# bytedance/particle-sfm

Measured on AMD Instinct MI355X. Metric: trajectory-points/s, higher is better.
Workload: dtype f32 sampling + f64 positions; 1 GPU; configs[1]: synthetic 100x(1920x1080) flow pairs, sample_ratio=2, flow_check + chaining + occlusion + id assignment, 1 sequence per GPU; frames=101, height=1080, width=1920, trajectories=2073277, parallelism=sequence-per-gpu x1, world_size=1

## Files before the change

### particle-sfm_amd/csrc/psfm_finalize.hip

```cpp
#include <cstring>
#include <stdio.h>
#include <rocprim/device/device_radix_sort.hpp>
#include <rocprim/device/device_scan.hpp>

#include "psfm_device.h"
#include "psfm_internal.h"

#define PSFM_BLOCK 256

__device__ __forceinline__ void psfm_collect_alive_body(
    const int* __restrict__ birth_frame, const int* __restrict__ birth_idx, PsfmCounters* __restrict__ ctr,
    PsfmShard* __restrict__ shards, unsigned long long* __restrict__ fin_keys, int* __restrict__ fin_lanes, int cap,
    int shard_cap, int last_time, int shift_b, int shift_d)
{
    __shared__ int s_cnt[PSFM_BLOCK / PSFM_WAVE];
    __shared__ int s_base;
    const int n_lanes = min(ctr->n_lanes, cap);
    if ((int)(blockIdx.x * PSFM_BLOCK) >= n_lanes) return;
    const int i = blockIdx.x * PSFM_BLOCK + threadIdx.x;
    int bf = -1;
    if (i < n_lanes) bf = birth_frame[i];
    const bool pending = bf <= -2;
    const bool alive = (bf >= 0) | pending;
    const int my_last = pending ? last_time - 1 : last_time;
// ... 276 lines not shown
        r[u] = t < lj ? log[(int64_t)(bj + t) * cap + col] : make_double2(0.0, 0.0);
    }
    if (tid < TILE_J) s_off[tid] = id0 + tid < n ? psfm_track_offset(pl, off, id0 + tid, hb, hl) : 0;
    for (int k0 = 0; k0 < maxlen; k0 += TILE_K) {
#pragma unroll
        for (int u = 0; u < NLD; ++u) tile[j][q + u * (PSFM_BLOCK / TILE_J)] = r[u];
        __syncthreads();
        if (k0 + TILE_K < maxlen) {
#pragma unroll
            for (int u = 0; u < NLD; ++u) {
                const int t = k0 + TILE_K + q + u * (PSFM_BLOCK / TILE_J);
                r[u] = t < lj ? log[(int64_t)(bj + t) * cap + col] : make_double2(0.0, 0.0);
            }
        }
        const int kk = tid & (TILE_K - 1);
        for (int jj = tid / TILE_K; jj < TILE_J; jj += PSFM_BLOCK / TILE_K) {
            const int t = k0 + kk;
            if (t < s_len[jj]) out[s_off[jj] + t] = tile[jj][kk];
        }
        __syncthreads();
    }
}

__global__ __launch_bounds__(PSFM_BLOCK) void psfm_gather_kernel(const double2* __restrict__ log, int64_t cap,
                                                                 const int* __restrict__ lanes,
                                                                 const int* __restrict__ birth,
                                                                 const int* __restrict__ len,
                                                                 const int64_t* __restrict__ off, int64_t n,
                                                                 double2* __restrict__ out, PsfmPlan pl)
{
    psfm_gather_body(log, cap, lanes, birth, len, off, n, out, pl);
}

__global__ __launch_bounds__(PSFM_BLOCK) void psfm_gather_delta_kernel(const float2* __restrict__ dlog, int64_t cap,
                                                                       const int* __restrict__ lanes,
                                                                       const int* __restrict__ birth,
                                                                       const int* __restrict__ len,
                                                                       const int64_t* __restrict__ off, int64_t n,
                                                                       const void* __restrict__ keys, int use32, int shift_b,
                                                                       int GW, int ratio, double2* __restrict__ out, PsfmPlan pl)
{
    __shared__ float2 dtile[TILE_J][TILE_K + 1];
    __shared__ double2 tile[TILE_J][TILE_K + 1];
    __shared__ double2 s_pos[TILE_J];
    __shared__ int s_lane[TILE_J], s_birth[TILE_J], s_len[TILE_J];
    __shared__ int64_t s_off[TILE_J];
    __shared__ int s_maxlen;
    const int tid = threadIdx.x;
    const int64_t id0 = (int64_t)blockIdx.x * TILE_J;
    int hb = 0, hl = 0;
    if (tid == 0) s_maxlen = 0;
    __syncthreads();
    if (tid < TILE_J) {
        const int64_t id = id0 + tid;
        const bool ok = id < n;
        int b = 0, l = 0, idx = -1;
        const int my_lane = ok ? lanes[id] : 0;
        if (ok) psfm_track_header(pl, birth, len, id, &b, &l, &idx);
        hb = b; hl = l;
        s_lane[tid] = my_lane;
        s_birth[tid] = b;
        s_len[tid] = l;
        if (ok) {
            atomicMax(&s_maxlen, l);
            if (idx < 0) {
                const unsigned long long mask = (1ull << shift_b) - 1ull;
                idx = (int)((use32 ? (unsigned long long)((const unsigned*)keys)[id] : ((const unsigned long long*)keys)[id]) & mask);
            }
            const int gy = idx / GW, gx = idx - gy * GW;
            s_pos[tid] = make_double2((double)(gx * ratio), (double)(gy * ratio));
        }
    }
    __syncthreads();
    const int maxlen = s_maxlen;
    const int j = tid & (TILE_J - 1);
    const int q = tid / TILE_J;
    constexpr int NLD = TILE_K * TILE_J / PSFM_BLOCK;
    const int lj = s_len[j];
    const int64_t col = s_lane[j];
    const int bj = s_birth[j];
    float2 r[NLD];
#pragma unroll
    for (int u = 0; u < NLD; ++u) {
        const int t = q + u * (PSFM_BLOCK / TILE_J);
        r[u] = (t >= 1 && t < lj) ? dlog[(int64_t)(bj + t - 1) * cap + col] : make_float2(0.f, 0.f);
    }
    if (tid < TILE_J) s_off[tid] = id0 + tid < n ? psfm_track_offset(pl, off, id0 + tid, hb, hl) : 0;
    for (int k0 = 0; k0 < maxlen; k0 += TILE_K) {
#pragma unroll
        for (int u = 0; u < NLD; ++u) dtile[j][q + u * (PSFM_BLOCK / TILE_J)] = r[u];
        __syncthreads();
        if (k0 + TILE_K < maxlen) {
#pragma unroll
            for (int u = 0; u < NLD; ++u) {
                const int t = k0 + TILE_K + q + u * (PSFM_BLOCK / TILE_J);
                r[u] = (t < lj) ? dlog[(int64_t)(bj + t - 1) * cap + col] : make_float2(0.f, 0.f);
            }
        }
        if (tid < TILE_J) {
            double2 pos = s_pos[tid];
            const int l = s_len[tid];
            float2 f[TILE_K];
#pragma unroll
            for (int k = 0; k < TILE_K; ++k) f[k] = dtile[tid][k];
#pragma unroll
            for (int k = 0; k < TILE_K; ++k) {
                const int t = k0 + k;
                if (t >= 1 && t < l) { pos.x = pos.x + (double)f[k].x; pos.y = pos.y + (double)f[k].y; }
                tile[tid][k] = pos;
            }
            s_pos[tid] = pos;
        }
        __syncthreads();
        const int kk = tid & (TILE_K - 1);
        for (int jj = tid / TILE_K; jj < TILE_J; jj += PSFM_BLOCK / TILE_K) {
            const int t = k0 + kk;
            if (t < s_len[jj]) out[s_off[jj] + t] = tile[jj][kk];
        }
        __syncthreads();
    }
}

static PsfmKeyFmt psfm_key_fmt(const PsfmTrackDims& d, unsigned* end_bit)
{
    PsfmKeyFmt f;
    f.shift_b = d.shift_b; f.shift_d = d.shift_d;
    const long long lmax = (long long)d.n_flows + 1;
    const long long tri_max = lmax * (lmax + 1) / 2 + lmax;
    int tri_bits = 1;
    while ((1ll << tri_bits) <= tri_max) ++tri_bits;
    f.use32 = (tri_bits + d.shift_b <= 32) ? 1 : 0;
    int tbits = 1;
    while ((1ll << tbits) < (long long)d.n_flows + 2) ++tbits;
    *end_bit = f.use32 ? (unsigned)(tri_bits + d.shift_b) : (unsigned)(d.shift_d + tbits);
    return f;
}

static bool psfm_own_sort(const PsfmKeyFmt& fmt, int64_t n)
{
    static const int on = getenv("PSFM_FIN_SORT") ? atoi(getenv("PSFM_FIN_SORT")) : 1;
    return on && fmt.use32 && n < (1ll << 31);
}
static bool psfm_records_in_first_half(const PsfmTrackDims& d, int64_t n)
{
    unsigned end_bit = 0;
    const PsfmKeyFmt fmt = psfm_key_fmt(d, &end_bit);
    return psfm_own_sort(fmt, n) && (psfm_sort_pairs32_passes(end_bit) % 2 == 0);
}

static psfm_status psfm_finalize_sorted(psfm_ctx* c, const PsfmTrackDims& d, int64_t n, int64_t npts, bool delta_log, hipStream_t s)
{
    psfm_status st;
// ... 31 lines not shown
    pl.birth_w = c->res_birth.as<int>(); pl.len_w = c->res_len.as<int>(); pl.off_w = c->res_off.as<int64_t>();
    if (plan_on && ng <= PSFM_PLAN_MAX_GROUPS && n < (1ll << 31)) {
        if ((st = c->scan_tmp.ensure((sizeof(int64_t) + sizeof(int)) * (size_t)ng)) != PSFM_OK) return st;
        int64_t* goff = c->scan_tmp.as<int64_t>();
        int* gstart = (int*)(goff + ng);
        const void* had = c->fin_marks.p;
        if ((st = c->fin_marks.ensure(sizeof(int) * (size_t)PSFM_PLAN_MAX_GROUPS)) != PSFM_OK) return st;
        if (!c->fin_marks_clean || had != c->fin_marks.p)
            PSFM_HIP(hipMemsetAsync(c->fin_marks.p, 0xff, sizeof(int) * (size_t)PSFM_PLAN_MAX_GROUPS, s));
        c->fin_marks_clean = false;
        hipLaunchKernelGGL(psfm_group_bounds_kernel, dim3((unsigned)((n + PSFM_BLOCK - 1) / PSFM_BLOCK)), dim3(PSFM_BLOCK), 0, s,
                           (const void*)c->sort_keys.p, n, fmt.use32, d.shift_b, d.shift_d, c->fin_marks.as<int>());
        hipLaunchKernelGGL(psfm_group_plan_kernel, dim3(1), dim3(PSFM_PLAN_BLOCK), 0, s, c->fin_marks.as<int>(), gstart, goff, (int)ng, n,
                           c->res_off.as<int64_t>() + n);
        PSFM_HIP(hipGetLastError());
        c->fin_marks_clean = true;
        pl.gstart = gstart; pl.goff = goff;
    } else {
        if ((st = c->scan_tmp.ensure(sizeof(int64_t) * (n + 1))) != PSFM_OK) return st;
        if (fmt.use32)
            hipLaunchKernelGGL(psfm_decode32_kernel, dim3((unsigned)((n + 1 + PSFM_BLOCK - 1) / PSFM_BLOCK)), dim3(PSFM_BLOCK), 0, s,
                               c->sort_keys.as<unsigned>(), n, d.shift_b, c->res_birth.as<int>(), c->res_len.as<int>(),
                               c->scan_tmp.as<int64_t>());
        else
            hipLaunchKernelGGL(psfm_decode_kernel, dim3((unsigned)((n + 1 + PSFM_BLOCK - 1) / PSFM_BLOCK)), dim3(PSFM_BLOCK), 0, s,
                               c->sort_keys.as<unsigned long long>(), n, d.shift_b, d.shift_d, c->res_birth.as<int>(),
                               c->res_len.as<int>(), c->scan_tmp.as<int64_t>());
        PSFM_HIP(hipGetLastError());
        PSFM_HIP(rocprim::exclusive_scan(c->sort_tmp.p, scan_bytes, c->scan_tmp.as<int64_t>(), c->res_off.as<int64_t>(),
                                         (int64_t)0, (size_t)(n + 1), rocprim::plus<int64_t>(), s));
    }
    c->res_n_points = npts;
    if ((st = c->res_xy.ensure(sizeof(double2) * (size_t)(npts > 0 ? npts : 1))) != PSFM_OK) return st;
    if (delta_log)
        hipLaunchKernelGGL(psfm_gather_delta_kernel, dim3((unsigned)((n + TILE_J - 1) / TILE_J)), dim3(PSFM_BLOCK), 0, s,
                           c->log.as<float2>(), d.cap, c->sort_lanes.as<int>(), c->res_birth.as<int>(),
                           c->res_len.as<int>(), c->res_off.as<int64_t>(), n, (const void*)c->sort_keys.p, fmt.use32,
                           d.shift_b, d.GW, d.ratio, c->res_xy.as<double2>(), pl);
    else
        hipLaunchKernelGGL(psfm_gather_kernel, dim3((unsigned)((n + TILE_J - 1) / TILE_J)), dim3(PSFM_BLOCK), 0, s,
                           c->log.as<double2>(), d.cap, c->sort_lanes.as<int>(), c->res_birth.as<int>(),
                           c->res_len.as<int>(), c->res_off.as<int64_t>(), n, c->res_xy.as<double2>(), pl);
    PSFM_HIP(hipGetLastError());
    return PSFM_OK;
}

psfm_status psfm_finalize(psfm_ctx* c, const PsfmTrackDims& d, hipStream_t s)
{
    PsfmCounters* ctr = c->counters.as<PsfmCounters>();
    PsfmShard* shards = c->shards.as<PsfmShard>();
    hipLaunchKernelGGL(psfm_collect_alive_kernel, dim3((unsigned)((d.cap + PSFM_BLOCK - 1) / PSFM_BLOCK)), dim3(PSFM_BLOCK),
                       0, s, c->birth_frame.as<int>(), c->birth_idx.as<int>(), ctr, shards,
                       c->fin_keys.as<unsigned long long>(), c->fin_lanes.as<int>(), (int)d.cap, d.shard_cap,
                       d.n_flows, d.shift_b, d.shift_d);
    PSFM_HIP(hipGetLastError());
    PsfmCounters* hc = (PsfmCounters*)c->host_pinned;
    PsfmShard* hs = (PsfmShard*)((char*)c->host_pinned + 512);
    PSFM_HIP(hipMemcpyAsync(hc, ctr, sizeof(PsfmCounters), hipMemcpyDeviceToHost, s));
    PSFM_HIP(hipMemcpyAsync(hs, shards, sizeof(PsfmShard) * PSFM_NSHARD, hipMemcpyDeviceToHost, s));
    PSFM_HIP(hipStreamSynchronize(s));
    PsfmShardOffsets so;
    int64_t n = 0, npts = 0;
    bool over = hc->overflow != 0;
    for (int k = 0; k < PSFM_NSHARD; ++k) npts += hs[k].points;
    for (int k = 0; k < PSFM_NSHARD; ++k) {
        if (hs[k].fin_cnt > d.shard_cap) over = true;
        so.count[k] = hs[k].fin_cnt > d.shard_cap ? d.shard_cap : hs[k].fin_cnt;
        so.start[k] = n;
        n += so.count[k];
    }
    if (over || hc->n_lanes > d.cap) {
// ... 334 lines not shown
```

### particle-sfm_amd/point_trajectory/_hip.py

```python
import ctypes
import os

_PKG = os.path.dirname(os.path.dirname(os.path.abspath(__file__)))
LIB_PATH = os.environ.get("PSFM_HIP_LIB", os.path.join(_PKG, "lib", "libpsfm_hip.so"))

PSFM_OK, PSFM_ERR_ARG, PSFM_ERR_HIP, PSFM_ERR_CAPACITY, PSFM_ERR_SOLVER = 0, 1, 2, 3, 4
PROF_KINDS = {"flow_check": 0, "chain_step": 1, "respawn": 2, "solver": 3, "finalize": 4}

EXPORTS = [
    "psfm_last_error", "psfm_version", "psfm_device_count", "psfm_ctx_create", "psfm_ctx_destroy",
    "psfm_ctx_set_capacity", "psfm_flow_check", "psfm_grid_sample", "psfm_optimize_location", "psfm_track",
    "psfm_connect",
    "psfm_result_device", "psfm_result_copy", "psfm_result_solve_stats", "psfm_ctx_set_profiling",
    "psfm_profile_get", "psfm_ctx_set_chain_mode", "psfm_window_sample", "psfm_result_filter", "psfm_result_filtered_copy",
    "psfm_ctx_set_solver", "psfm_solver_counters", "psfm_traj_to_matches", "psfm_matches_copy",
    "psfm_shard_begin", "psfm_shard_step", "psfm_shard_solve_export", "psfm_shard_solve_control", "psfm_shard_solve_restore",
    "psfm_shard_solve_writeback", "psfm_shard_solve_record", "psfm_shard_finish", "psfm_result_keys",
    "psfm_shard_solve_control_async", "psfm_shard_window_state", "psfm_shard_peek_stall", "psfm_shard_frame",
    "psfm_shard_solve_control_chain_async", "psfm_shard_solve_poll", "psfm_shard_solve_local", "psfm_shard_solve_redo_local", "psfm_connect_batch", "psfm_solver_launches", "psfm_ctx_set_resident_budget", "psfm_resident_capacity", "psfm_load_flo_stack",
    "psfm_path_consistency_eval", "psfm_sort_records",
    "psfm_shard_peer_area", "psfm_shard_peer_epoch", "psfm_shard_peer_open", "psfm_shard_peer_connect", "psfm_shard_solve_blocks", "psfm_shard_solve_peer",
    "psfm_labels_begin", "psfm_labels_merge_window", "psfm_labels_finish", "psfm_labels_device", "psfm_labels_copy", "psfm_labels_to_matches",
]

# ... 77 lines not shown
    L.psfm_labels_to_matches.argtypes = [vp, i32, i32, i32, ctypes.POINTER(i64), ctypes.POINTER(i64), ctypes.POINTER(i64), vp]
    L.psfm_shard_begin.argtypes = [vp, i32, i32, i32, i32, i64, i64, i32, vp, i64, vp]
    L.psfm_shard_step.argtypes = [vp, vp, vp, i32, vp]
    L.psfm_shard_solve_export.argtypes = [vp, vp, vp, vp, vp, i32, i32, i32, vp, vp]
    L.psfm_shard_frame.argtypes = [vp, vp, vp, vp, vp, vp, i32, i32, vp, vp]
    L.psfm_shard_solve_control.argtypes = [vp, i32, i32, i32, vp, ctypes.POINTER(ctypes.c_int32), ctypes.POINTER(ctypes.c_int32),
                                           ctypes.POINTER(SolveStats), vp]
    L.psfm_shard_solve_control_async.argtypes = [vp, i32, i32, vp, vp]
    L.psfm_shard_solve_control_chain_async.argtypes = [vp, i32, i32, vp, vp]
    L.psfm_shard_solve_poll.argtypes = [vp, ctypes.POINTER(ctypes.c_int32), ctypes.POINTER(SolveStats), vp]
    L.psfm_shard_solve_local.argtypes = [vp, vp, vp, vp, vp, i32, i32, vp]
    L.psfm_shard_peer_area.argtypes = [vp, ctypes.POINTER(vp), vp, vp]
    L.psfm_shard_peer_open.argtypes = [vp, vp, i32, ctypes.POINTER(vp)]
    L.psfm_shard_peer_epoch.argtypes = [vp, ctypes.POINTER(ctypes.c_uint32), i32, vp]
    L.psfm_shard_peer_connect.argtypes = [vp, i32, i32, ctypes.POINTER(vp), ctypes.POINTER(ctypes.c_int32)]
    L.psfm_shard_solve_blocks.argtypes = [vp, ctypes.POINTER(ctypes.c_int32)]
    L.psfm_shard_solve_peer.argtypes = [vp, vp, vp, vp, vp, i32, ctypes.c_uint32, vp]
    L.psfm_shard_solve_redo_local.argtypes = [vp, vp, vp, vp, vp, i32, i32, ctypes.POINTER(SolveStats), vp]
    L.psfm_shard_window_state.argtypes = [vp, i32, i32, ctypes.POINTER(SolveStats), ctypes.POINTER(ctypes.c_int32), vp]
    L.psfm_shard_peek_stall.argtypes = [vp, ctypes.POINTER(ctypes.c_int32)]
    L.psfm_shard_solve_restore.argtypes = [vp, i32, vp]
    L.psfm_shard_solve_writeback.argtypes = [vp, i32, ctypes.POINTER(SolveStats), vp]
    L.psfm_shard_solve_record.argtypes = [vp, ctypes.POINTER(SolveStats)]
    L.psfm_shard_finish.argtypes = [vp, ctypes.POINTER(TrackInfo), vp]
    L.psfm_result_keys.argtypes = [vp, i32, i32, vp, vp]
    L.psfm_profile_get.argtypes = [vp, i32, ctypes.POINTER(f64), ctypes.POINTER(i64)]
    for name in EXPORTS:
        if name != "psfm_last_error":
            getattr(L, name).restype = i32
    _lib = L
    return L


def check(status):
    if status != PSFM_OK:
        raise PsfmError(status, lib().psfm_last_error().decode("utf-8", "replace"))


class Context:

    def __init__(self, device=0):
        self._h = ctypes.c_void_p()
        check(lib().psfm_ctx_create(int(device), ctypes.byref(self._h)))
        self.device = int(device)
        self.resident_budget = 0

    @property
    def handle(self):
        return self._h

    def set_capacity(self, lane_factor, traj_factor):
        check(lib().psfm_ctx_set_capacity(self._h, float(lane_factor), float(traj_factor)))

    def set_chain_mode(self, mode):
        check(lib().psfm_ctx_set_chain_mode(self._h, int(mode)))

    def set_solver(self, mode, k=0):
        check(lib().psfm_ctx_set_solver(self._h, int(mode), int(k)))

    def set_resident_budget(self, blocks):
        check(lib().psfm_ctx_set_resident_budget(self._h, int(blocks)))
        self.resident_budget = int(blocks)

    def resident_capacity(self):
        n = ctypes.c_int32()
        check(lib().psfm_resident_capacity(self._h, ctypes.byref(n)))
# ... 92 lines not shown
```

### particle-sfm_amd/csrc/psfm_persist.hip

```cpp
#include <hip/hip_ext.h>
#include <stdlib.h>

#include "psfm_internal.h"
#include "psfm_chain.h"

#define PP_BLOCK 256
#define PP_NW (PP_BLOCK / PSFM_WAVE)
#define PP_PROBE 8
#ifndef PP_PRE_WAVES
#define PP_PRE_WAVES 4
#endif
#ifndef PP_KEEP
#define PP_KEEP 0
#endif
#ifndef PP_FC_AHEAD
#define PP_FC_AHEAD 4
#endif
#ifndef PP_FC_FAST
#define PP_FC_FAST 0
#endif
#define PP_GUESTS 32
#ifndef PP_WHATIF
#define PP_WHATIF 0
#endif
// ... 140 lines not shown
            if (p >= P) break;
            uint8_t o;
#if PP_FC_FAST
            {
                const float X = __fadd_rn((float)x, fv[k].x), Y = __fadd_rn((float)y, fv[k].y);
                const PsfmTaps t = psfm_taps_t<true>(X, Y, q.cw, q.ch, q.rcw, q.rch, q.H, q.W);
                const bool interior = (t.x0 >= 0) & (t.x0 + 1 < q.W) & (t.y0 >= 0) & (t.y0 + 1 < q.H);
                if (__builtin_amdgcn_ballot_w64(!interior) == 0ull) o = psfm_flow_check_px_interior(B, X, Y, fv[k], t, q);
                else { float e; int xb = x, yb = y; asm volatile("" : "+v"(xb), "+v"(yb)); o = psfm_flow_check_px<false>(B, xb, yb, fv[k], q, &e); }
            }
#else
            float e;
            o = psfm_flow_check_px<false>(B, x, y, fv[k], q, &e);
#endif
            psfm_coh_st(O + p, o);
            x += 256;
            while (x >= a.W) { x -= a.W; ++y; }
        }
    }
}

__device__ __forceinline__ int psfm_vblock(const PsfmPersistArgs& a)
{
    const int b = (int)blockIdx.x;
    return (a.xcd_per > 0 && b < 8 * a.xcd_per) ? (b & 7) * a.xcd_per + (b >> 3) : b;
}

struct PsfmEntry { int kind, ex, host; };

template <int R>
__global__ __launch_bounds__(PP_BLOCK) PP_WAVES void psfm_chain_persist_kernel(PsfmPersistArgs a)
{
    __shared__ int s_births[PP_NW], s_adopt[PP_NW], s_pend[PP_NW];
    __shared__ int s_new_g[PP_BLOCK];
    __shared__ int s_ad_tid[PP_BLOCK];
    __shared__ int s_pend_tid[PP_BLOCK];
    __shared__ double2 s_xp[PP_BLOCK];
    __shared__ int s_xg[PP_BLOCK];
    __shared__ int s_xf[PP_BLOCK];
    __shared__ int s_gi[PP_BLOCK];
    __shared__ int s_npts[PP_BLOCK];
    __shared__ int s_seg_start[PP_PROBE + 1], s_seg_end[PP_PROBE + 1];
    __shared__ int s_nseg, s_base_free, s_ok, s_alive_any[2], s_rec_cnt, s_done;
    __shared__ double2 s_gp[PP_GUESTS];
    __shared__ int s_gbf[PP_GUESTS];
    __shared__ int s_ggi[PP_GUESTS];
    __shared__ int s_glive[PP_GUESTS], s_gfree[PP_GUESTS], s_nglive, s_ngfree;

    int tid = threadIdx.x;
    int L = psfm_vblock(a) * PP_BLOCK + tid;
    const int ratio = R > 0 ? R : a.ratio;
    const int shard = blockIdx.x % PSFM_NSHARD;
    const size_t P = (size_t)a.H * a.W;

    int bf = PP_POOLED;
    double2 p = make_double2(0.0, 0.0);
    s_gi[tid] = L;
    s_npts[tid] = 0;
    if (L < a.G) {
        const int gy = (int)psfm_fastdiv((unsigned)L, a.gwdiv), gx = L - gy * a.GW;
        p = make_double2((double)(gx * ratio), (double)(gy * ratio));
        bf = 0;
        s_npts[tid] = 1;
    }
    s_xf[tid] = 0;
    if (tid < PP_GUESTS) s_gbf[tid] = -1;
    if (tid == 0) { s_rec_cnt = 0; s_alive_any[0] = 0; s_alive_any[1] = 0; s_done = 0; }
    int fc_next = 0;
    if (a.fc) {
        for (; fc_next < 2 && fc_next < a.n_flows; ++fc_next) psfm_fc_slice(a, fc_next, tid);
        __builtin_amdgcn_s_waitcnt(0);
    }
    __syncthreads();
    if (tid / PSFM_WAVE == PP_NW - 1) psfm_bar_arrive(a, shard, 0, tid & (PSFM_WAVE - 1));
    if (a.fc) {
        if (tid == 0) s_ok = psfm_bar_wait(a, shard, 0) ? 1 : 0;
        __syncthreads();
        if (!s_ok) return;
    }

    for (int t = 0; t < a.n_flows; ++t) {
        asm volatile("" : "+v"(tid));
        L = psfm_vblock(a) * PP_BLOCK + tid;
        const int lane = tid & (PSFM_WAVE - 1), wave = tid / PSFM_WAVE;
        PsfmFrameView v;
        v.flow = a.flows + (size_t)t * P; v.occ = a.occ + (size_t)t * a.occ_pitch;
        v.H = a.H; v.W = a.W; v.cw = a.cw; v.ch = a.ch; v.rcw = a.rcw; v.rch = a.rch; v.ratio = a.ratio; v.GW = a.GW; v.GH = a.GH; v.rdiv = a.rdiv;
        v.blocked_cur = a.maps + (size_t)(t % 3) * a.G; v.stamp_cur = 1;
        float2* dlog_t = a.dlog + (size_t)t * a.cap;
        const int cur = t & 1, prev = cur ^ 1;

        PP_TL(0);
        const bool live = bf >= 0;
        bool any_alive = false;
        int npts = 0;
        auto own_step = [&](const PsfmFrameView& vs, float2* slab, int s, const PsfmStepLoads& ld, bool mine, bool& alive_any) {
            PsfmStep s1;
            s1.alive = true;
            if (mine) s1 = psfm_step_finish(vs, p, ld);
            const int slot1 = psfm_record_slot(&s_rec_cnt, !s1.alive);
            if (mine) {
                if (s1.alive) {
                    if (PP_CHK(L, a.cap, 1)) slab[L] = s1.flow;
                    psfm_block_grid<R, PP_COH_MARKS>(vs, (int)s1.next.x, (int)s1.next.y);
                    p = s1.next;
                    alive_any = true;
                    ++npts;
                } else {
                    psfm_put_record(a, slot1, psfm_key(s, bf, s_gi[tid], a.shift_b, a.shift_d), L);
                    bf = PP_PEND;
                    p = make_double2(0.0, 0.0);
                }
            }
        };
        PsfmStepLoads l1 = psfm_step_issue(v, p);

        auto do_E = [&]() { own_step(v, dlog_t, t, l1, live, any_alive); };
        const bool e_first = wave < PP_PRE_WAVES;
        if (e_first) do_E();

        if (a.fc) {
            const unsigned* flag = a.bar + (65 + shard) * 32;
            const int fc_lim = t + PP_FC_AHEAD < a.n_flows ? t + PP_FC_AHEAD : a.n_flows;
            while (fc_next < fc_lim) {
                if (__builtin_amdgcn_readfirstlane((int)psfm_coh_ld(flag)) >= t + 1 || (PP_WHATIF & 32)) break;
                psfm_fc_slice(a, fc_next, tid);
                ++fc_next;
            }
        }
        if (tid == 0) s_ok = (PP_WHATIF & 4) ? 1 : (psfm_bar_wait(a, shard, t) ? 1 : 0);
        __syncthreads();
        if (!s_ok) return;

#ifndef PP_NO_SETPRIO
        __builtin_amdgcn_s_setprio(3);
#endif
        PP_TL(1);
        const bool poll = t > 0 && bf == PP_POOLED && !(PP_WHATIF & 8);
        const bool gridpt = t > 0 && L < a.G && !(PP_WHATIF & 8);
        uint8_t* map_prev = a.maps + (size_t)((t + 2) % 3) * a.G;
        unsigned sv = 0, byte = 0;
        unsigned long long h0 = 0, h1 = 0, h2 = ~0ull;
        if (t > 0 && blockIdx.x == 0 && tid < PSFM_NSHARD) sv = psfm_coh_ld(a.survsh + (prev * PSFM_NSHARD + tid) * 32);
        if (gridpt) byte = psfm_coh_ld(map_prev + L);
        if (poll) {
            const unsigned long long* h = a.handoff + (size_t)L * 3;
            h0 = psfm_coh_ld(h); h1 = psfm_coh_ld(h + 1); h2 = psfm_coh_ld(h + 2);
        }

        if (!e_first) do_E();

        const unsigned long long svm = __ballot(sv == (unsigned)t);
        bool birth = false;
        if (gridpt) {
            if (byte != 0) psfm_coh_st(map_prev + L, (uint8_t)0);
            birth = byte == 0;
            if (L == 0 && svm == 0ull) birth = ((0 + 1) * (0 + 1) + 0 * 0) > ratio * ratio;
            if (PP_WHATIF & 1) birth = false;
        }
        bool adopted = false;
        if (poll) {
            const int tag = (int)(h2 >> 32);
            if ((tag >> 1) == t - 1 && !(PP_WHATIF & 1)) {
                if (tag & 1) {
                    adopted = true;
                    s_xp[tid] = make_double2(__longlong_as_double((long long)h0), __longlong_as_double((long long)h1));
                    s_xg[tid] = (int)(unsigned)h2;
                } else {
                    bf = PP_PEND;
                }
            }
        }
        const bool pend = (bf == PP_PEND) & !live;
        const unsigned long long bm = __ballot(birth), am = __ballot(adopted), pm = __ballot(pend);
        if (lane == 0) { s_births[wave] = __popcll(bm); s_adopt[wave] = __popcll(am); s_pend[wave] = __popcll(pm); }
        if (birth) s_new_g[wave * PSFM_WAVE + psfm_rank_in(bm)] = L;
        if (adopted) s_ad_tid[wave * PSFM_WAVE + psfm_rank_in(am)] = tid;
        if (pend) s_pend_tid[wave * PSFM_WAVE + psfm_rank_in(pm)] = tid;
        if (wave == 0) {
            const int gb = tid < PP_GUESTS ? s_gbf[tid] : -1;
            const bool gl = gb >= 0, gf = (tid < PP_GUESTS) & (gb < 0);
            const unsigned long long glm = __ballot(gl), gfm = __ballot(gf);
            if (lane == 0) { s_nglive = __popcll(glm); s_ngfree = __popcll(gfm); }
            if (gl) s_glive[psfm_rank_in(glm)] = tid;
            if (gf) s_gfree[psfm_rank_in(gfm)] = tid;
        }
        __syncthreads();

        PP_TL(2);
        int nb = 0, nad = 0, npd = 0, my_pend_before = 0;
#pragma unroll
        for (int w = 0; w < PP_NW; ++w) {
            if (w == wave) my_pend_before = npd;
            nb += s_births[w]; nad += s_adopt[w]; npd += s_pend[w];
        }
        const int matched = nb < npd ? nb : npd;
        const int ngl = s_nglive;
        const int gmatched = (nb - matched) < s_ngfree ? (nb - matched) : s_ngfree;
        const int n2 = nb + nad + ngl;

        for (int base = 0; base == 0 || base < n2; base += PP_BLOCK) {
            const int k = base + tid;
            PsfmEntry e;
            e.kind = 0; e.ex = -1; e.host = -1;
            if (k < nb) {
                int before = 0, pb = 0;
#pragma unroll
                for (int w = 0; w < PP_NW; ++w) {
                    const int c = s_births[w], pc = s_pend[w];
                    if (k >= before && k < before + c) e.ex = s_new_g[w * PSFM_WAVE + (k - before)];
                    if (k >= pb && k < pb + pc) e.host = s_pend_tid[w * PSFM_WAVE + (k - pb)];
                    before += c; pb += pc;
                }
                e.kind = 1;
            } else if (k < nb + nad) {
                const int kk = k - nb;
                int before = 0;
#pragma unroll
                for (int w = 0; w < PP_NW; ++w) {
                    const int c = s_adopt[w];
                    if (kk >= before && kk < before + c) e.ex = s_ad_tid[w * PSFM_WAVE + (kk - before)];
                    before += c;
                }
                e.kind = 2;
            } else if (k < n2) {
                e.ex = s_glive[k - nb - nad];
                e.kind = 3;
            }
            PsfmStepLoads l2 = {};
            if (e.kind != 0) {
                double2 q;
                if (e.kind == 1) {
                    const int gy = (int)psfm_fastdiv((unsigned)e.ex, a.gwdiv), gx = e.ex - gy * a.GW;
                    q = make_double2((double)(gx * ratio), (double)(gy * ratio));
                } else if (e.kind == 2) {
                    q = s_xp[e.ex];
                } else {
                    q = s_gp[e.ex];
                }
                l2 = psfm_step_issue(v, q);
            }
#ifdef PSFM_TIMELINE
            if (base == 0 && tid == 0 && t == g_pp_tl_frame) {
// ... 66 lines not shown
                if (e.kind == 1) {
                    const int gy = (int)psfm_fastdiv((unsigned)e.ex, a.gwdiv), gx = e.ex - gy * a.GW;
                    q = make_double2((double)(gx * ratio), (double)(gy * ratio));
                    bfk = t; gik = e.ex;
                    if (k < matched) {
                        col = psfm_vblock(a) * PP_BLOCK + e.host;
                    } else if (k < matched + gmatched) {
                        gs = s_gfree[k - matched];
                        col = a.cap_main + blockIdx.x * PP_GUESTS + gs;
                    } else {
                        const int* free_pop = a.free_stack + (size_t)cur * a.free_cap * PSFM_NSHARD;
                        const int qq = k - matched - gmatched;
                        int j = 0, pv = 0;
                        while (j < s_nseg - 1 && qq >= s_seg_end[j]) { pv = s_seg_end[j]; ++j; }
                        const int st = s_seg_start[j];
                        if (st >= 0) (void)PP_CHK(st - (qq - pv), 2 * a.free_cap * PSFM_NSHARD, 9);
                        col = st >= 0 ? psfm_coh_ld(free_pop + (st - (qq - pv))) : (-(st + 1) + (qq - pv));
                        if (col >= a.cap_main) col = -1;
                    }
                } else if (e.kind == 2) {
                    q = s_xp[e.ex];
                    bfk = t - 1; gik = s_xg[e.ex];
                    col = psfm_vblock(a) * PP_BLOCK + e.ex;
                } else {
                    q = s_gp[e.ex];
                    bfk = s_gbf[e.ex]; gik = s_ggi[e.ex];
                    col = a.cap_main + blockIdx.x * PP_GUESTS + e.ex;
                }
                if (col >= 0) {
                    (void)PP_CHK(col, a.cap, 2);
                    const PsfmStep s2 = psfm_step_finish(v, q, l2);
                    if (e.kind == 1) ++npts;
                    if (s2.alive) {
                        if (PP_CHK(col, a.cap, 3)) dlog_t[col] = s2.flow;
                        psfm_block_grid<R, PP_COH_MARKS>(v, (int)s2.next.x, (int)s2.next.y);
                        any_alive = true;
                        ++npts;
                    } else {
                        const int slot = atomicAdd(&s_rec_cnt, 1);
                        psfm_put_record(a, slot, psfm_key(t, bfk, gik, a.shift_b, a.shift_d), col);
                    }
                    if (e.kind == 1) {
                        const bool popped = k >= matched + gmatched;
                        if (popped && s2.alive && t == a.n_flows - 1) {
                            const int slot = atomicAdd(&s_rec_cnt, 1);
                            psfm_put_record(a, slot, psfm_key(a.n_flows, t, e.ex, a.shift_b, a.shift_d), col);
                        }
                        if (k < matched) {
                            s_xp[e.host] = s2.next; s_xg[e.host] = e.ex; s_xf[e.host] = s2.alive ? 1 : 2;
                        } else if (gs >= 0) {
                            if (s2.alive) { s_gp[gs] = s2.next; s_ggi[gs] = e.ex; s_gbf[gs] = t; }
                        } else if (PP_CHK(col, a.cap_main, 8)) {
                            unsigned long long* h = a.handoff + (size_t)col * 3;
                            psfm_coh_st(h, (unsigned long long)__double_as_longlong(s2.next.x));
                            psfm_coh_st(h + 1, (unsigned long long)__double_as_longlong(s2.next.y));
                            psfm_coh_st(h + 2, (unsigned long long)(unsigned)e.ex |
                                                   ((unsigned long long)(unsigned)(2 * t + (s2.alive ? 1 : 0)) << 32));
                        }
                    } else if (e.kind == 2) {
                        if (s2.alive) s_xp[e.ex] = s2.next;
                        s_xf[e.ex] = s2.alive ? 1 : 2;
                    } else {
                        if (s2.alive) s_gp[e.ex] = s2.next;
                        else s_gbf[e.ex] = -1;
                    }
                } else {
                    atomicOr(&a.ctr->overflow, 4);
// ... 10 lines not shown
            if (f != 0) {
                s_xf[tid] = 0;
                if (f == 1) {
                    bf = adopted ? t - 1 : t;
                    s_gi[tid] = s_xg[tid];
                    p = s_xp[tid];
                } else {
                    bf = PP_PEND;
                }
            }
        }
        if (tid == 0 && s_alive_any[t & 1]) { psfm_coh_st(a.survsh + (cur * PSFM_NSHARD + shard) * 32, (unsigned)(t + 1)); s_alive_any[t & 1] = 0; }
        if (a.fc) {
            const int need = t + 3 < a.n_flows ? t + 3 : a.n_flows;
            if (!(PP_WHATIF & 16)) for (; fc_next < need; ++fc_next) psfm_fc_slice(a, fc_next, tid);
        }
        if (!(PP_WHATIF & 2)) asm volatile("s_waitcnt vmcnt(0) lgkmcnt(0)" ::: "memory");
        PP_TL(6);
        {
            int last_wave = 0;
            if (lane == 0) last_wave = atomicAdd(&s_done, 1) == PP_NW - 1 ? 1 : 0;
            last_wave = __builtin_amdgcn_readfirstlane(last_wave);
            if (last_wave) {
                if (lane == 0) s_done = 0;
                PP_TL(7);
                psfm_bar_arrive(a, shard, t + 1, lane);
            }
        }
#ifndef PP_NO_SETPRIO
        __builtin_amdgcn_s_setprio(0);
#endif
    }

    const int lane = tid & (PSFM_WAVE - 1), wave = tid / PSFM_WAVE;
    {
        const bool alive = bf >= 0;
        const int slot = psfm_record_slot(&s_rec_cnt, alive);
        if (alive) psfm_put_record(a, slot, psfm_key(a.n_flows, bf, s_gi[tid], a.shift_b, a.shift_d), L);
        if (tid < PP_GUESTS && s_gbf[tid] >= 0) {
            const int gslot = atomicAdd(&s_rec_cnt, 1);
            psfm_put_record(a, gslot, psfm_key(a.n_flows, s_gbf[tid], s_ggi[tid], a.shift_b, a.shift_d),
                            a.cap_main + blockIdx.x * PP_GUESTS + tid);
        }
    }
    {
        __shared__ int s_pts[PP_NW];
        int w = s_npts[tid];
#pragma unroll
        for (int o = 32; o > 0; o >>= 1) w += __shfl_down(w, o);
        if (lane == 0) s_pts[wave] = w;
        __syncthreads();
        if (tid == 0) {
            int tot = 0;
            for (int j = 0; j < PP_NW; ++j) tot += s_pts[j];
            const int c = s_rec_cnt;
            a.seg_info[blockIdx.x] = make_int2(c < a.seg_cap ? c : a.seg_cap, tot);
        }
    }
}

__global__ __launch_bounds__(256) void psfm_persist_init_kernel(PsfmCounters* ctr, PsfmShard* shards, int G,
                                                                unsigned long long* maps64, size_t n_maps64,
                                                                unsigned long long* bar64, size_t n_bar64,
                                                                unsigned long long* handoff, size_t n_handoff)
{
    const size_t i = (size_t)blockIdx.x * 256 + threadIdx.x, stride = (size_t)gridDim.x * 256;
// ... 105 lines not shown
```

Baseline: 20.91 billion trajectory-points/s.

## Parallelize delta prefix-sum across four waves with exactness-checked fallback

The delta-gather kernel now runs the per-track running sum across all four waves of the block. Each wave accumulates its quarter of a chunk in registers, and the waves combine through a small shared-memory partial-total array. This replaces the previous approach where only the first 64 threads did a serial scan of the whole chunk. A per-value exponent check keeps the result bit-identical to the serial order: if any flow value could make the reassociated double sums inexact, the whole block falls back to the old serial path. The change also adds debug counters for fallback rounds, an optional reversed block order, and env knobs, at the cost of an extra block-wide vote and added code complexity.

```diff
diff --git a/particle-sfm_amd/csrc/psfm_finalize.hip b/particle-sfm_amd/csrc/psfm_finalize.hip
--- a/particle-sfm_amd/csrc/psfm_finalize.hip
+++ b/particle-sfm_amd/csrc/psfm_finalize.hip
@@ -332,22 +332,53 @@
     psfm_gather_body(log, cap, lanes, birth, len, off, n, out, pl);
 }
 
+#define PSFM_FIN_QK (TILE_K * TILE_J / PSFM_BLOCK)
+static_assert(PSFM_BLOCK / TILE_J == 4 && PSFM_FIN_QK * 4 == TILE_K, "four quarters of a chunk, one per wave");
+static_assert(sizeof(float2) * TILE_K <= sizeof(double2) * (TILE_K / 2), "the raw flows of a row fit its upper half");
+
+__device__ unsigned long long g_fin_rounds[64][16];
+static int g_fin_count_all = 0;
+extern "C" int psfm_debug_gather_rounds(unsigned long long* out_host, int reset)
+{
+    static unsigned long long h[64][16];
+    if (hipDeviceSynchronize() != hipSuccess) return 1;
+    if (out_host) {
+        if (hipMemcpyFromSymbol(h, HIP_SYMBOL(g_fin_rounds), sizeof(h)) != hipSuccess) return 1;
+        out_host[0] = out_host[1] = 0ull;
+        for (int k = 0; k < 64; ++k) { out_host[0] += h[k][0]; out_host[1] += h[k][1]; }
+    }
+    if (reset) {
+        memset(h, 0, sizeof(h));
+        if (hipMemcpyToSymbol(HIP_SYMBOL(g_fin_rounds), h, sizeof(h)) != hipSuccess) return 1;
+        g_fin_count_all = 1;
+    }
+    return 0;
+}
+
+__device__ __forceinline__ int psfm_flow_inexact(float v, int emin)
+{
+    const unsigned a = __float_as_uint(v) & 0x7fffffffu;
+    const int e = (int)(a >> 23);
+    return (a != 0u) & ((e + __builtin_ctz(a | 0x800000u) < emin) | (a >= 0x7f800000u));
+}
+
 __global__ __launch_bounds__(PSFM_BLOCK) void psfm_gather_delta_kernel(const float2* __restrict__ dlog, int64_t cap,
                                                                        const int* __restrict__ lanes,
                                                                        const int* __restrict__ birth,
                                                                        const int* __restrict__ len,
                                                                        const int64_t* __restrict__ off, int64_t n,
                                                                        const void* __restrict__ keys, int use32, int shift_b,
-                                                                       int GW, int ratio, double2* __restrict__ out, PsfmPlan pl)
-{
-    __shared__ float2 dtile[TILE_J][TILE_K + 1];
+                                                                       int GW, int ratio, double2* __restrict__ out, PsfmPlan pl,
+                                                                       int emin, int flip, int count_all)
+{
     __shared__ double2 tile[TILE_J][TILE_K + 1];
+    __shared__ double2 s_tot[PSFM_BLOCK / TILE_J][TILE_J];
     __shared__ double2 s_pos[TILE_J];
     __shared__ int s_lane[TILE_J], s_birth[TILE_J], s_len[TILE_J];
     __shared__ int64_t s_off[TILE_J];
     __shared__ int s_maxlen;
     const int tid = threadIdx.x;
-    const int64_t id0 = (int64_t)blockIdx.x * TILE_J;
+    const int64_t id0 = (int64_t)(flip ? gridDim.x - 1u - blockIdx.x : blockIdx.x) * TILE_J;
     int hb = 0, hl = 0;
     if (tid == 0) s_maxlen = 0;
     __syncthreads();
@@ -361,6 +392,7 @@
         s_lane[tid] = my_lane;
         s_birth[tid] = b;
         s_len[tid] = l;
+        double2 p0 = make_double2(0.0, 0.0);
         if (ok) {
             atomicMax(&s_maxlen, l);
             if (idx < 0) {
@@ -368,45 +400,72 @@
                 idx = (int)((use32 ? (unsigned long long)((const unsigned*)keys)[id] : ((const unsigned long long*)keys)[id]) & mask);
             }
             const int gy = idx / GW, gx = idx - gy * GW;
-            s_pos[tid] = make_double2((double)(gx * ratio), (double)(gy * ratio));
-        }
+            p0 = make_double2((double)(gx * ratio), (double)(gy * ratio));
+        }
+        s_pos[tid] = p0;
     }
     __syncthreads();
     const int maxlen = s_maxlen;
     const int j = tid & (TILE_J - 1);
     const int q = tid / TILE_J;
-    constexpr int NLD = TILE_K * TILE_J / PSFM_BLOCK;
+    constexpr int NLD = PSFM_FIN_QK;
     const int lj = s_len[j];
     const int64_t col = s_lane[j];
     const int bj = s_birth[j];
     float2 r[NLD];
 #pragma unroll
     for (int u = 0; u < NLD; ++u) {
-        const int t = q + u * (PSFM_BLOCK / TILE_J);
+        const int t = q * NLD + u;
         r[u] = (t >= 1 && t < lj) ? dlog[(int64_t)(bj + t - 1) * cap + col] : make_float2(0.f, 0.f);
     }
     if (tid < TILE_J) s_off[tid] = id0 + tid < n ? psfm_track_offset(pl, off, id0 + tid, hb, hl) : 0;
+    unsigned n_rounds = 0, n_serial = 0;
     for (int k0 = 0; k0 < maxlen; k0 += TILE_K) {
-#pragma unroll
-        for (int u = 0; u < NLD; ++u) dtile[j][q + u * (PSFM_BLOCK / TILE_J)] = r[u];
-        __syncthreads();
+        const double2 p = s_pos[j];
+        int bad = emin < 0;
+        double2 loc[NLD];
+        double2 run = make_double2(0.0, 0.0);
+#pragma unroll
+        for (int u = 0; u < NLD; ++u) {
+            bad |= psfm_flow_inexact(r[u].x, emin) | psfm_flow_inexact(r[u].y, emin);
+            run.x = run.x + (double)r[u].x; run.y = run.y + (double)r[u].y;
+            loc[u] = run;
+        }
+        s_tot[q][j] = run;
+        const int serial = __syncthreads_or(bad);
+        ++n_rounds;
+        if (serial) {
+            ++n_serial;
+            float2* raw = (float2*)&tile[j][TILE_K / 2];
+#pragma unroll
+            for (int u = 0; u < NLD; ++u) raw[q * NLD + u] = r[u];
+            __syncthreads();
+        }
         if (k0 + TILE_K < maxlen) {
 #pragma unroll
             for (int u = 0; u < NLD; ++u) {
-                const int t = k0 + TILE_K + q + u * (PSFM_BLOCK / TILE_J);
+                const int t = k0 + TILE_K + q * NLD + u;
                 r[u] = (t < lj) ? dlog[(int64_t)(bj + t - 1) * cap + col] : make_float2(0.f, 0.f);
             }
         }
-        if (tid < TILE_J) {
-            double2 pos = s_pos[tid];
-            const int l = s_len[tid];
-            float2 f[TILE_K];
-#pragma unroll
-            for (int k = 0; k < TILE_K; ++k) f[k] = dtile[tid][k];
+        if (!serial) {
+            double2 base = p;
+            if (q > 0) {
+                double2 pre = s_tot[0][j];
+                for (int w = 1; w < q; ++w) { const double2 v = s_tot[w][j]; pre.x = pre.x + v.x; pre.y = pre.y + v.y; }
+                base.x = p.x + pre.x; base.y = p.y + pre.y;
+            }
+#pragma unroll
+            for (int u = 0; u < NLD; ++u) tile[j][q * NLD + u] = make_double2(base.x + loc[u].x, base.y + loc[u].y);
+            if (q == PSFM_BLOCK / TILE_J - 1) s_pos[j] = make_double2(base.x + loc[NLD - 1].x, base.y + loc[NLD - 1].y);
+        } else if (tid < TILE_J) {
+            double2 pos = p;
+            const float2* raw = (const float2*)&tile[tid][TILE_K / 2];
 #pragma unroll
             for (int k = 0; k < TILE_K; ++k) {
+                const float2 f = raw[k];
                 const int t = k0 + k;
-                if (t >= 1 && t < l) { pos.x = pos.x + (double)f[k].x; pos.y = pos.y + (double)f[k].y; }
+                if (t >= 1 && t < lj) { pos.x = pos.x + (double)f.x; pos.y = pos.y + (double)f.y; }
                 tile[tid][k] = pos;
             }
             s_pos[tid] = pos;
@@ -418,6 +477,10 @@
             if (t < s_len[jj]) out[s_off[jj] + t] = tile[jj][kk];
         }
         __syncthreads();
+    }
+    if (tid == 0) {
+        if (n_serial) atomicAdd(&g_fin_rounds[blockIdx.x & 63][0], (unsigned long long)n_serial);
+        if (count_all) atomicAdd(&g_fin_rounds[blockIdx.x & 63][1], (unsigned long long)n_rounds);
     }
 }
 
@@ -515,11 +578,16 @@
     }
     c->res_n_points = npts;
     if ((st = c->res_xy.ensure(sizeof(double2) * (size_t)(npts > 0 ? npts : 1))) != PSFM_OK) return st;
-    if (delta_log)
+    if (delta_log) {
+        static const int exact_on = getenv("PSFM_FIN_EXACT") ? atoi(getenv("PSFM_FIN_EXACT")) : 1;
+        static const int long_first = getenv("PSFM_FIN_LONGFIRST") ? atoi(getenv("PSFM_FIN_LONGFIRST")) : 0;
+        int B = 0;
+        while ((1 << B) < (d.H > d.W ? d.H : d.W)) ++B;
         hipLaunchKernelGGL(psfm_gather_delta_kernel, dim3((unsigned)((n + TILE_J - 1) / TILE_J)), dim3(PSFM_BLOCK), 0, s,
                            c->log.as<float2>(), d.cap, c->sort_lanes.as<int>(), c->res_birth.as<int>(),
                            c->res_len.as<int>(), c->res_off.as<int64_t>(), n, (const void*)c->sort_keys.p, fmt.use32,
-                           d.shift_b, d.GW, d.ratio, c->res_xy.as<double2>(), pl);
+                           d.shift_b, d.GW, d.ratio, c->res_xy.as<double2>(), pl, exact_on ? 98 + B : -1, long_first, g_fin_count_all);
+    }
     else
         hipLaunchKernelGGL(psfm_gather_kernel, dim3((unsigned)((n + TILE_J - 1) / TILE_J)), dim3(PSFM_BLOCK), 0, s,
                            c->log.as<double2>(), d.cap, c->sort_lanes.as<int>(), c->res_birth.as<int>(),
diff --git a/particle-sfm_amd/point_trajectory/_hip.py b/particle-sfm_amd/point_trajectory/_hip.py
--- a/particle-sfm_amd/point_trajectory/_hip.py
+++ b/particle-sfm_amd/point_trajectory/_hip.py
@@ -133,6 +133,15 @@
     return L
 
 
+def gather_rounds(reset=False):
+    out = (ctypes.c_ulonglong * 2)()
+    fn = lib().psfm_debug_gather_rounds
+    fn.argtypes = [ctypes.POINTER(ctypes.c_ulonglong), ctypes.c_int]
+    if fn(out, 1 if reset else 0) != 0:
+        raise RuntimeError("psfm_debug_gather_rounds failed")
+    return int(out[0]), int(out[1])
+
+
 def check(status):
     if status != PSFM_OK:
         raise PsfmError(status, lib().psfm_last_error().decode("utf-8", "replace"))
```

Result: no change. 21.09 billion trajectory-points/s (median of 3 runs) (+0.9%).

## Stage flow deltas in LDS and store dlog in quad-interleaved layout

Applied to the files above, without the earlier changes.

The persistent chaining kernel now buffers per-lane flow deltas for four consecutive frames in shared memory and flushes them as two 16-byte stores into a frame-quad-interleaved dlog layout, instead of writing one float2 per frame to a per-frame slab. The gather-delta kernel is rewritten to match: each track-owner thread loads its deltas directly as float4 quads into registers with a phase offset and prefetches the next tile, dropping the separate shared transposition tile. Several shared index arrays shrink to uint8 to make room for the staging buffers. The aim is fewer, wider global transactions on both write and read, at the cost of more LDS use and added flush and phase bookkeeping, which could reduce occupancy of the persistent kernel.

```diff
diff --git a/particle-sfm_amd/csrc/psfm_finalize.hip b/particle-sfm_amd/csrc/psfm_finalize.hip
--- a/particle-sfm_amd/csrc/psfm_finalize.hip
+++ b/particle-sfm_amd/csrc/psfm_finalize.hip
@@ -340,82 +340,77 @@
                                                                        const void* __restrict__ keys, int use32, int shift_b,
                                                                        int GW, int ratio, double2* __restrict__ out, PsfmPlan pl)
 {
-    __shared__ float2 dtile[TILE_J][TILE_K + 1];
-    __shared__ double2 tile[TILE_J][TILE_K + 1];
-    __shared__ double2 s_pos[TILE_J];
-    __shared__ int s_lane[TILE_J], s_birth[TILE_J], s_len[TILE_J];
-    __shared__ int64_t s_off[TILE_J];
-    __shared__ int s_maxlen;
+    constexpr int TJ = TILE_J, TK = TILE_K, GD_QUADS = TK / 4;
+    __shared__ double2 tile[TJ][TK + 1];
+    __shared__ int s_ph[TJ], s_len[TJ];
+    __shared__ int64_t s_off[TJ];
+    __shared__ int s_span;
     const int tid = threadIdx.x;
-    const int64_t id0 = (int64_t)blockIdx.x * TILE_J;
-    int hb = 0, hl = 0;
-    if (tid == 0) s_maxlen = 0;
-    __syncthreads();
-    if (tid < TILE_J) {
+    const int64_t id0 = (int64_t)blockIdx.x * TJ;
+    if (tid == 0) s_span = 0;
+    __syncthreads();
+    double2 pos = make_double2(0.0, 0.0);
+    int l = 0, ph = 0, last_q = -1;
+    const float4* src = (const float4*)dlog;
+    float4 r[2 * GD_QUADS];
+    if (tid < TJ) {
         const int64_t id = id0 + tid;
         const bool ok = id < n;
-        int b = 0, l = 0, idx = -1;
+        int b = 0, idx = -1;
         const int my_lane = ok ? lanes[id] : 0;
         if (ok) psfm_track_header(pl, birth, len, id, &b, &l, &idx);
-        hb = b; hl = l;
-        s_lane[tid] = my_lane;
-        s_birth[tid] = b;
+        ph = b & 3;
+        if (l >= 2) last_q = (ph + l - 2) >> 2;
+        src += ((int64_t)(b >> 2) * cap + my_lane) * 2;
+#pragma unroll
+        for (int i = 0; i < GD_QUADS; ++i) {
+            const bool in = i <= last_q;
+            r[2 * i] = in ? src[(int64_t)i * cap * 2] : make_float4(0.f, 0.f, 0.f, 0.f);
+            r[2 * i + 1] = in ? src[(int64_t)i * cap * 2 + 1] : make_float4(0.f, 0.f, 0.f, 0.f);
+        }
+        s_ph[tid] = ph;
         s_len[tid] = l;
         if (ok) {
-            atomicMax(&s_maxlen, l);
+            atomicMax(&s_span, ph + l);
             if (idx < 0) {
                 const unsigned long long mask = (1ull << shift_b) - 1ull;
                 idx = (int)((use32 ? (unsigned long long)((const unsigned*)keys)[id] : ((const unsigned long long*)keys)[id]) & mask);
             }
             const int gy = idx / GW, gx = idx - gy * GW;
-            s_pos[tid] = make_double2((double)(gx * ratio), (double)(gy * ratio));
-        }
-    }
-    __syncthreads();
-    const int maxlen = s_maxlen;
-    const int j = tid & (TILE_J - 1);
-    const int q = tid / TILE_J;
-    constexpr int NLD = TILE_K * TILE_J / PSFM_BLOCK;
-    const int lj = s_len[j];
-    const int64_t col = s_lane[j];
-    const int bj = s_birth[j];
-    float2 r[NLD];
-#pragma unroll
-    for (int u = 0; u < NLD; ++u) {
-        const int t = q + u * (PSFM_BLOCK / TILE_J);
-        r[u] = (t >= 1 && t < lj) ? dlog[(int64_t)(bj + t - 1) * cap + col] : make_float2(0.f, 0.f);
-    }
-    if (tid < TILE_J) s_off[tid] = id0 + tid < n ? psfm_track_offset(pl, off, id0 + tid, hb, hl) : 0;
-    for (int k0 = 0; k0 < maxlen; k0 += TILE_K) {
-#pragma unroll
-        for (int u = 0; u < NLD; ++u) dtile[j][q + u * (PSFM_BLOCK / TILE_J)] = r[u];
+            pos = make_double2((double)(gx * ratio), (double)(gy * ratio));
+        }
+        s_off[tid] = ok ? psfm_track_offset(pl, off, id, b, l) : 0;
+    }
+    __syncthreads();
+    const int span = s_span;
+    for (int k0 = 0; k0 < span; k0 += TK) {
+        if (tid < TJ) {
+            const int q0 = (k0 + TK) >> 2;
+#pragma unroll
+            for (int h = 0; h < 2; ++h) {
+#pragma unroll
+                for (int k = h * (TK / 2); k < (h + 1) * (TK / 2); ++k) {
+                    const int t = k0 + k - ph;
+                    tile[tid][k] = pos;
+                    const float4 v = r[k >> 1];
+                    const float fx = (k & 1) ? v.z : v.x, fy = (k & 1) ? v.w : v.y;
+                    if (t >= 0 && t < l - 1) { pos.x = pos.x + (double)fx; pos.y = pos.y + (double)fy; }
+                }
+                if (k0 + TK < span) {
+#pragma unroll
+                    for (int i = h * (GD_QUADS / 2); i < (h + 1) * (GD_QUADS / 2); ++i) {
+                        const bool in = q0 + i <= last_q;
+                        r[2 * i] = in ? src[(int64_t)(q0 + i) * cap * 2] : make_float4(0.f, 0.f, 0.f, 0.f);
+                        r[2 * i + 1] = in ? src[(int64_t)(q0 + i) * cap * 2 + 1] : make_float4(0.f, 0.f, 0.f, 0.f);
+                    }
+                }
+            }
+        }
         __syncthreads();
-        if (k0 + TILE_K < maxlen) {
-#pragma unroll
-            for (int u = 0; u < NLD; ++u) {
-                const int t = k0 + TILE_K + q + u * (PSFM_BLOCK / TILE_J);
-                r[u] = (t < lj) ? dlog[(int64_t)(bj + t - 1) * cap + col] : make_float2(0.f, 0.f);
-            }
-        }
-        if (tid < TILE_J) {
-            double2 pos = s_pos[tid];
-            const int l = s_len[tid];
-            float2 f[TILE_K];
-#pragma unroll
-            for (int k = 0; k < TILE_K; ++k) f[k] = dtile[tid][k];
-#pragma unroll
-            for (int k = 0; k < TILE_K; ++k) {
-                const int t = k0 + k;
-                if (t >= 1 && t < l) { pos.x = pos.x + (double)f[k].x; pos.y = pos.y + (double)f[k].y; }
-                tile[tid][k] = pos;
-            }
-            s_pos[tid] = pos;
-        }
-        __syncthreads();
-        const int kk = tid & (TILE_K - 1);
-        for (int jj = tid / TILE_K; jj < TILE_J; jj += PSFM_BLOCK / TILE_K) {
-            const int t = k0 + kk;
-            if (t < s_len[jj]) out[s_off[jj] + t] = tile[jj][kk];
+        const int kk = tid & (TK - 1);
+        for (int jj = tid / TK; jj < TJ; jj += PSFM_BLOCK / TK) {
+            const int t = k0 + kk - s_ph[jj];
+            if (t >= 0 && t < s_len[jj]) out[s_off[jj] + t] = tile[jj][kk];
         }
         __syncthreads();
     }
diff --git a/particle-sfm_amd/csrc/psfm_persist.hip b/particle-sfm_amd/csrc/psfm_persist.hip
--- a/particle-sfm_amd/csrc/psfm_persist.hip
+++ b/particle-sfm_amd/csrc/psfm_persist.hip
@@ -196,9 +196,9 @@
 __global__ __launch_bounds__(PP_BLOCK) PP_WAVES void psfm_chain_persist_kernel(PsfmPersistArgs a)
 {
     __shared__ int s_births[PP_NW], s_adopt[PP_NW], s_pend[PP_NW];
-    __shared__ int s_new_g[PP_BLOCK];
-    __shared__ int s_ad_tid[PP_BLOCK];
-    __shared__ int s_pend_tid[PP_BLOCK];
+    __shared__ uint8_t s_new_g[PP_BLOCK];
+    __shared__ uint8_t s_ad_tid[PP_BLOCK];
+    __shared__ uint8_t s_pend_tid[PP_BLOCK];
     __shared__ double2 s_xp[PP_BLOCK];
     __shared__ int s_xg[PP_BLOCK];
     __shared__ int s_xf[PP_BLOCK];
@@ -209,7 +209,10 @@
     __shared__ double2 s_gp[PP_GUESTS];
     __shared__ int s_gbf[PP_GUESTS];
     __shared__ int s_ggi[PP_GUESTS];
-    __shared__ int s_glive[PP_GUESTS], s_gfree[PP_GUESTS], s_nglive, s_ngfree;
+    __shared__ uint8_t s_glive[PP_GUESTS], s_gfree[PP_GUESTS];
+    __shared__ int s_nglive, s_ngfree;
+    __shared__ float2 s_stage[4][PP_BLOCK + PP_GUESTS];
+    __shared__ unsigned s_stflag[PP_BLOCK + PP_GUESTS];
 
     int tid = threadIdx.x;
     int L = psfm_vblock(a) * PP_BLOCK + tid;
@@ -228,7 +231,8 @@
         s_npts[tid] = 1;
     }
     s_xf[tid] = 0;
-    if (tid < PP_GUESTS) s_gbf[tid] = -1;
+    s_stflag[tid] = 0u;
+    if (tid < PP_GUESTS) { s_gbf[tid] = -1; s_stflag[PP_BLOCK + tid] = 0u; }
     if (tid == 0) { s_rec_cnt = 0; s_alive_any[0] = 0; s_alive_any[1] = 0; s_done = 0; }
     int fc_next = 0;
     if (a.fc) {
@@ -242,6 +246,27 @@
         __syncthreads();
         if (!s_ok) return;
     }
+
+    auto flush_quad = [&](int sc, int col, int quad) {
+        const unsigned m = s_stflag[sc];
+        if (m == 0u) return;
+        s_stflag[sc] = 0u;
+        if (!PP_CHK(col, a.cap, 1)) return;
+        float2* dst = a.dlog + ((size_t)quad * a.cap + col) * 4;
+        if (m == 0x01010101u) {
+            const float2 f0 = s_stage[0][sc], f1 = s_stage[1][sc], f2 = s_stage[2][sc], f3 = s_stage[3][sc];
+            ((float4*)dst)[0] = make_float4(f0.x, f0.y, f1.x, f1.y);
+            ((float4*)dst)[1] = make_float4(f2.x, f2.y, f3.x, f3.y);
+        } else {
+#pragma unroll
+            for (int k = 0; k < 4; ++k)
+                if ((m >> (8 * k)) & 1u) dst[k] = s_stage[k][sc];
+        }
+    };
+    auto flush_mine = [&](int quad) {
+        flush_quad(tid, L, quad);
+        if (tid < PP_GUESTS) flush_quad(PP_BLOCK + tid, a.cap_main + blockIdx.x * PP_GUESTS + tid, quad);
+    };
 
     for (int t = 0; t < a.n_flows; ++t) {
         asm volatile("" : "+v"(tid));
@@ -251,21 +276,21 @@
         v.flow = a.flows + (size_t)t * P; v.occ = a.occ + (size_t)t * a.occ_pitch;
         v.H = a.H; v.W = a.W; v.cw = a.cw; v.ch = a.ch; v.rcw = a.rcw; v.rch = a.rch; v.ratio = a.ratio; v.GW = a.GW; v.GH = a.GH; v.rdiv = a.rdiv;
         v.blocked_cur = a.maps + (size_t)(t % 3) * a.G; v.stamp_cur = 1;
-        float2* dlog_t = a.dlog + (size_t)t * a.cap;
         const int cur = t & 1, prev = cur ^ 1;
+        auto stage = [&](int sc, float2 f) { s_stage[t & 3][sc] = f; ((uint8_t*)s_stflag)[sc * 4 + (t & 3)] = 1; };
 
         PP_TL(0);
         const bool live = bf >= 0;
         bool any_alive = false;
         int npts = 0;
-        auto own_step = [&](const PsfmFrameView& vs, float2* slab, int s, const PsfmStepLoads& ld, bool mine, bool& alive_any) {
+        auto own_step = [&](const PsfmFrameView& vs, int s, const PsfmStepLoads& ld, bool mine, bool& alive_any) {
             PsfmStep s1;
             s1.alive = true;
             if (mine) s1 = psfm_step_finish(vs, p, ld);
             const int slot1 = psfm_record_slot(&s_rec_cnt, !s1.alive);
             if (mine) {
                 if (s1.alive) {
-                    if (PP_CHK(L, a.cap, 1)) slab[L] = s1.flow;
+                    stage(tid, s1.flow);
                     psfm_block_grid<R, PP_COH_MARKS>(vs, (int)s1.next.x, (int)s1.next.y);
                     p = s1.next;
                     alive_any = true;
@@ -278,8 +303,9 @@
             }
         };
         PsfmStepLoads l1 = psfm_step_issue(v, p);
-
-        auto do_E = [&]() { own_step(v, dlog_t, t, l1, live, any_alive); };
+        if ((t & 3) == 0 && t > 0) flush_mine((t >> 2) - 1);
+
+        auto do_E = [&]() { own_step(v, t, l1, live, any_alive); };
         const bool e_first = wave < PP_PRE_WAVES;
         if (e_first) do_E();
 
@@ -338,16 +364,16 @@
         const bool pend = (bf == PP_PEND) & !live;
         const unsigned long long bm = __ballot(birth), am = __ballot(adopted), pm = __ballot(pend);
         if (lane == 0) { s_births[wave] = __popcll(bm); s_adopt[wave] = __popcll(am); s_pend[wave] = __popcll(pm); }
-        if (birth) s_new_g[wave * PSFM_WAVE + psfm_rank_in(bm)] = L;
-        if (adopted) s_ad_tid[wave * PSFM_WAVE + psfm_rank_in(am)] = tid;
-        if (pend) s_pend_tid[wave * PSFM_WAVE + psfm_rank_in(pm)] = tid;
+        if (birth) s_new_g[wave * PSFM_WAVE + psfm_rank_in(bm)] = (uint8_t)tid;
+        if (adopted) s_ad_tid[wave * PSFM_WAVE + psfm_rank_in(am)] = (uint8_t)tid;
+        if (pend) s_pend_tid[wave * PSFM_WAVE + psfm_rank_in(pm)] = (uint8_t)tid;
         if (wave == 0) {
             const int gb = tid < PP_GUESTS ? s_gbf[tid] : -1;
             const bool gl = gb >= 0, gf = (tid < PP_GUESTS) & (gb < 0);
             const unsigned long long glm = __ballot(gl), gfm = __ballot(gf);
             if (lane == 0) { s_nglive = __popcll(glm); s_ngfree = __popcll(gfm); }
-            if (gl) s_glive[psfm_rank_in(glm)] = tid;
-            if (gf) s_gfree[psfm_rank_in(gfm)] = tid;
+            if (gl) s_glive[psfm_rank_in(glm)] = (uint8_t)tid;
+            if (gf) s_gfree[psfm_rank_in(gfm)] = (uint8_t)tid;
         }
         __syncthreads();
 
@@ -372,7 +398,7 @@
 #pragma unroll
                 for (int w = 0; w < PP_NW; ++w) {
                     const int c = s_births[w], pc = s_pend[w];
-                    if (k >= before && k < before + c) e.ex = s_new_g[w * PSFM_WAVE + (k - before)];
+                    if (k >= before && k < before + c) e.ex = psfm_vblock(a) * PP_BLOCK + s_new_g[w * PSFM_WAVE + (k - before)];
                     if (k >= pb && k < pb + pc) e.host = s_pend_tid[w * PSFM_WAVE + (k - pb)];
                     before += c; pb += pc;
                 }
@@ -505,7 +531,9 @@
                     const PsfmStep s2 = psfm_step_finish(v, q, l2);
                     if (e.kind == 1) ++npts;
                     if (s2.alive) {
-                        if (PP_CHK(col, a.cap, 3)) dlog_t[col] = s2.flow;
+                        const int sc = e.kind == 1 ? (k < matched ? e.host : gs >= 0 ? PP_BLOCK + gs : -1) : e.kind == 2 ? e.ex : PP_BLOCK + e.ex;
+                        if (sc >= 0) stage(sc, s2.flow);
+                        else if (PP_CHK(col, a.cap, 3)) a.dlog[((size_t)(t >> 2) * a.cap + col) * 4 + (t & 3)] = s2.flow;
                         psfm_block_grid<R, PP_COH_MARKS>(v, (int)s2.next.x, (int)s2.next.y);
                         any_alive = true;
                         ++npts;
@@ -582,6 +610,7 @@
 #endif
     }
 
+    if (a.n_flows > 0) flush_mine((a.n_flows - 1) >> 2);
     const int lane = tid & (PSFM_WAVE - 1), wave = tid / PSFM_WAVE;
     {
         const bool alive = bf >= 0;
```

Result: slower. 21.13 billion trajectory-points/s before, 20.77 billion trajectory-points/s after (-1.7%).
